# mmurooka/SMPLpp

Measured on AMD Instinct MI355X. Metric: SMPL FK evals/s + IK iters/s, batch 1024 frames, 1/2/4/8 MI355X, higher is better.
Workload: dtype f32 (exact operands: every fp32 value as three bf16 pieces = fp32's 24 bits on the bf16 matrix pipe, fp32 accumulate; fp32 VALU skinning)

## Files before the change

### smplpp_amd/csrc/fk.hip

```cpp
#include "common.h"
#include "pose_math.h"
#ifdef POSE_STAMP
namespace smplpp_hip
{
__device__ unsigned long long g_pose_stamps[16];
}
#define PST(i) if(blockIdx.x == 512 && threadIdx.x == 0) smplpp_hip::g_pose_stamps[i] = __builtin_amdgcn_s_memtime()
#define PSTC(i) if(blockIdx.x == 512 && threadIdx.x == 192) smplpp_hip::g_pose_stamps[i] = __builtin_amdgcn_s_memtime()
extern "C" int smplpp_debug_pose_stamps(unsigned long long * out)
{
  return (int)hipMemcpyFromSymbol(out, HIP_SYMBOL(smplpp_hip::g_pose_stamps), sizeof(unsigned long long) * 16);
}
#endif
#include "pose_body.h"
#include "staging.h"
#include "trace.h"

namespace smplpp_hip
{
typedef float f32x16 __attribute__((ext_vector_type(16)));
typedef _Float16 f16x8 __attribute__((ext_vector_type(8)));

__global__ __launch_bounds__(256) void pose_kernel(PoseArgs a)
{
// ... 172 lines not shown
static hipError_t launch_skin_w(const smplpp_model * m, int64_t n, const float * theta, float * verts, float * rest,
                                hipStream_t st)
{
  switch(m->maxw)
  {
    case 4:
      return launch_skin<FT, 4>(m, n, theta, verts, rest, st);
    case 8:
      return launch_skin<FT, 8>(m, n, theta, verts, rest, st);
    default:
      return launch_skin<FT, NJ>(m, n, theta, verts, rest, st);
  }
}

hipError_t launch_skin_bf16x3(const smplpp_model * m, int64_t n, const float * theta, float * verts, float * rest, hipStream_t st);
hipError_t launch_skin_f16x2(const smplpp_model * m, int64_t n, const float * theta, float * verts, float * rest, hipStream_t st);
hipError_t launch_skin_exact(const smplpp_model * m, int64_t n, const float * theta, float * verts, float * rest, hipStream_t st);

PoseArgs fk_pose_args(smplpp_model * m, int64_t n, const float * beta, const float * theta, float * joints, float * poserot, float * xforms44,
                      bool with_ops)
{
  Workspace & ws = m->ws;
  PoseArgs pa;
  pa.beta = beta;
  pa.theta = theta;
  pa.J0 = m->J0.get();
  pa.JS = m->JS.get();
  pa.JSp = m->JSp.get();
  pa.parent = m->parent.get();
  pa.lvl_off = m->lvl.get();
  pa.lvl_joint = m->lvl.get() + NJ + 1;
  pa.nlev = m->nlev;
// ... 51 lines not shown
    {
      int64_t cnt = (int64_t)KP * (ldA - n);
      zero_pad_kernel<<<dim3((unsigned)((cnt + 255) / 256)), dim3(256), 0, st>>>(ws.AT.as<float>(), ldA, n);
    }
    PoseArgs pa = fk_pose_args(m, n, beta, theta, joints, poserot, xforms44, false);
    pa.AT = ws.AT.as<float>();
    pa.ldA = ldA;
    pa.gscale = 1.0f;
    pa.range_flag = nullptr;
    pose_kernel<<<dim3((unsigned)n), dim3(256), 0, st>>>(pa);
  }
  HIP_TRY(hipGetLastError());
  return SMPLPP_OK;
}

static int fk_skin_device(smplpp_model * m, char form, int64_t n, const float * theta, float * verts, float * rest, hipStream_t st)
{
  if(verts || rest)
  {
    hipEvent_t e0 = nullptr, e1 = nullptr;
    if(m->profiling)
    {
      HIP_TRY(hipEventCreate(&e0));
      if(hipError_t ee = hipEventCreate(&e1); ee != hipSuccess)
      {
        (void)hipEventDestroy(e0);
        return hip_fail(ee, "hipEventCreate", __FILE__, __LINE__);
      }
      m->prof_events.push_back(e0);
      m->prof_events.push_back(e1);
      HIP_TRY(hipEventRecord(e0, st));
    }
    if(form == 'e')
      HIP_TRY(launch_skin_exact(m, n, theta, verts, rest, st));
    else if(form == 'h')
      HIP_TRY(launch_skin_f16x2(m, n, theta, verts, rest, st));
    else if(form == 'b')
      HIP_TRY(launch_skin_bf16x3(m, n, theta, verts, rest, st));
    else if(n <= 32)
      HIP_TRY(launch_skin_w<1>(m, n, theta, verts, rest, st));
    else
      HIP_TRY(launch_skin_w<2>(m, n, theta, verts, rest, st));
    if(m->profiling) HIP_TRY(hipEventRecord(e1, st));
  }
  return SMPLPP_OK;
}

int fk_device(smplpp_model * m, int64_t n, const float * beta, const float * theta, float * verts, float * joints,
              float * xforms44, float * rest, float * poserot, hipStream_t st, int range_slot, int * range_word, char form_override = 0)
{
  const char form = launch_form(m, range_slot, form_override);
  int rc = fk_pose_device(m, form, n, beta, theta, joints, xforms44, poserot, st, range_word ? range_word : m->range_flag.get() + range_slot,
                          verts || rest);
  if(rc) return rc;
  return fk_skin_device(m, form, n, theta, verts, rest, st);
}
}

using namespace smplpp_hip;

extern "C" int smplpp_profile_enable(smplpp_model * m, int enable)
{
  if(!m) return fail(SMPLPP_ERR_INVALID, "smplpp_profile_enable: null model");
  m->profiling = enable != 0;
  return SMPLPP_OK;
}

extern "C" int smplpp_profile_read(smplpp_model * m, int64_t * launches, double * mean_ms)
{
  if(!m || !launches || !mean_ms) return fail(SMPLPP_ERR_INVALID, "smplpp_profile_read: null argument");
// ... 77 lines not shown
```

### smplpp_amd/csrc/ik.hip

```cpp
#include "ik_types.h"
#include "ik_eval.h"
#include "ik_solve.h"
#include "ik_proj.h"
#include "vposer_state.h"

#include <algorithm>
#include <chrono>
#include <cstdlib>

using namespace smplpp_hip;

struct smplpp_ik
{
  smplpp_model * m = nullptr;
  smplpp_vposer * vp = nullptr;
  int64_t n = 0, K = 0;
  int64_t frame_base = 0;
  int theta_dim = TD75;
  TaskArrays ta{};
  float *theta = nullptr, *beta = nullptr, *theta25 = nullptr, *vjac = nullptr;
  float *verts = nullptr, *rest = nullptr, *joints = nullptr, *poserot = nullptr, *pts = nullptr;
  double *e = nullptr, *J = nullptr, *Jl = nullptr, *e2 = nullptr, *xout = nullptr;
  int *skip = nullptr, *status = nullptr, *sticky = nullptr, *list_cnt = nullptr, *list_f = nullptr;
  int * range_word = nullptr;
  int32_t * roles = nullptr;
  float * list_d = nullptr;
  std::vector<DevPtr<void>> owned;
  bool have_eval = false;
  int64_t last_D = 0;
  hipStream_t side = nullptr;
  hipEvent_t ev_fork = nullptr, ev_join = nullptr;
  bool phi_locked = false;
  bool side_pending = false;
  int * dbg_buf = nullptr;
  unsigned * sig = nullptr;
  unsigned tick_fork = 0, tick_join = 0, tick_done = 0;
  bool use_flags = false;
  double last_enqueue_us = 0.0;
  bool latent_split = false;
  bool latent_split_default = false;
  bool exact = false;
  StatePtr<VPoserJxWork> jxw;
  bool jac_ahead = false;
  bool dbg_sync = false, overlap_ok = true;
  int dbg_stop = 0;
  int64_t scan_blocks = 1536;
  int scan_form = -1;
  float * vbuf[2] = {nullptr, nullptr};
  int vcur = 0;
  ~smplpp_ik()
  {
    (void)hipSetDevice(m->device);
// ... 97 lines not shown
  if(K > PROJ_MAXK) return fail(SMPLPP_ERR_INVALID, "smplpp_ik_create: at most 48 tasks per frame are supported");
  if(TD75 + 2 * K + NB > MAXD)
    return fail(SMPLPP_ERR_INVALID, "smplpp_ik_create: too many tasks for the in-LDS solver (75 + 2K + 10 must be <= 181)");
  HIP_TRY(hipSetDevice(m->device));
  std::unique_ptr<smplpp_ik> s(new smplpp_ik());
  s->m = m;
  s->vp = vposer;
  s->n = n;
  s->K = K;
  s->theta_dim = vposer ? TD44 : TD75;
  {
    const char * e;
    s->dbg_sync = getenv("SMPLPP_DEBUG_SYNC") != nullptr;
    if((e = getenv("SMPLPP_IK_DBG_STOP"))) s->dbg_stop = atoi(e);
    if((e = getenv("SMPLPP_IK_OVERLAP"))) s->overlap_ok = e[0] != '0';
    if(s->dbg_sync) s->overlap_ok = false;
    s->scan_blocks = (n >= 256 && n < 512) ? 2 * n : 1536;
    if(n >= 512 && K <= 8 && (m->F + 767) / 768 <= 32) s->scan_blocks = n * ((m->F + 767) / 768);
    if((e = getenv("SMPLPP_SCAN_BLOCKS"))) s->scan_blocks = atoll(e);
    if((e = getenv("SMPLPP_SCAN_FORM"))) s->scan_form = atoi(e);
    s->latent_split = vposer != nullptr && n <= 128 && s->dbg_stop == 0;
    if((e = getenv("SMPLPP_IK_LATENT_SPLIT"))) s->latent_split = vposer != nullptr && e[0] != '0' && s->dbg_stop == 0;
  }
  const size_t nk = (size_t)n * K;
  const size_t Dmax = TD75 + 2 * K + NB;
  HIP_TRY(dalloc(s.get(), &s->ta.face, nk));
  HIP_TRY(dalloc(s.get(), &s->ta.vw, nk * 3));
  HIP_TRY(dalloc(s.get(), &s->ta.tang, nk * 6));
  HIP_TRY(dalloc(s.get(), &s->ta.tpos, nk * 3));
  HIP_TRY(dalloc(s.get(), &s->ta.tnrm, nk * 3));
// ... 13 lines not shown
  HIP_TRY(dalloc(s.get(), &s->rest, (size_t)n * m->V * 3));
  HIP_TRY(dalloc(s.get(), &s->joints, (size_t)n * NJ * 3));
  HIP_TRY(dalloc(s.get(), &s->poserot, (size_t)n * NJ * 9));
  HIP_TRY(dalloc(s.get(), &s->pts, nk * 3));
  HIP_TRY(dalloc(s.get(), &s->e, nk * 4));
  HIP_TRY(dalloc(s.get(), &s->J, nk * 4 * Dmax));
  HIP_TRY(dalloc(s.get(), &s->e2, (size_t)n));
  HIP_TRY(dalloc(s.get(), &s->xout, (size_t)n * Dmax));
  HIP_TRY(dalloc(s.get(), &s->roles, roles.size()));
  HIP_TRY(dalloc(s.get(), &s->list_cnt, nk));
  HIP_TRY(dalloc(s.get(), &s->list_d, nk * PROJ_LIST));
  HIP_TRY(dalloc(s.get(), &s->list_f, nk * PROJ_LIST));
  HIP_TRY(dalloc(s.get(), &s->skip, (size_t)n));
  HIP_TRY(dalloc(s.get(), &s->status, (size_t)n));
  HIP_TRY(dalloc(s.get(), &s->sticky, (size_t)n));
  HIP_TRY(dalloc(s.get(), &s->range_word, 1));
  s->ta.flags = s->sticky;
  if(vposer)
  {
    HIP_TRY(dalloc(s.get(), &s->Jl, nk * 4 * Dmax));
    HIP_TRY(dalloc(s.get(), &s->vjac, (size_t)n * 63 * 32));
  }
  auto grid = [](size_t c) { return dim3((unsigned)((c + 255) / 256)); };
  HIP_TRY(hipMemset(s->ta.face, 0, sizeof(int32_t) * nk));
  fill_f32_kernel<<<grid(nk * 3), 256>>>(s->ta.vw, 1.0f / 3.0f, nk * 3);
  fill_f32_kernel<<<grid(nk * 6), 256>>>(s->ta.tang, 0.0f, nk * 6);
  fill_f32_kernel<<<grid(nk * 3), 256>>>(s->ta.tpos, 0.0f, nk * 3);
  fill_nrm_kernel<<<grid(nk * 3), 256>>>(s->ta.tnrm, nk * 3);
  fill_f32_kernel<<<grid(nk), 256>>>(s->ta.posw, 1.0f, nk);
  fill_f32_kernel<<<grid(nk), 256>>>(s->ta.nrmw, 1.0f, nk);
  fill_f32_kernel<<<grid(nk), 256>>>(s->ta.philim, 0.04f, nk);
  fill_f32_kernel<<<grid(nk), 256>>>(s->ta.noff, 0.0f, nk);
  HIP_TRY(hipMemset(s->theta, 0, sizeof(float) * n * s->theta_dim));
  HIP_TRY(hipMemset(s->theta25, 0, sizeof(float) * n * 75));
  HIP_TRY(hipMemset(s->beta, 0, sizeof(float) * n * NB));
  HIP_TRY(hipMemset(s->skip, 0, sizeof(int) * n));
  HIP_TRY(hipMemcpy(s->roles, roles.data(), sizeof(int32_t) * roles.size(), hipMemcpyHostToDevice));
  HIP_TRY(hipMemset(s->list_cnt, 0, sizeof(int) * nk));
  HIP_TRY(hipMemset(s->status, 0, sizeof(int) * n));
  HIP_TRY(hipMemset(s->sticky, 0, sizeof(int) * n));
  HIP_TRY(hipMemset(s->range_word, 0, sizeof(int)));
  s->verts = s->vbuf[0];
  HIP_TRY(hipStreamCreateWithFlags(&s->side, hipStreamNonBlocking));
  HIP_TRY(hipEventCreateWithFlags(&s->ev_fork, hipEventDisableTiming));
  HIP_TRY(hipEventCreateWithFlags(&s->ev_join, hipEventDisableTiming));
  {
    HIP_TRY(dalloc(s.get(), &s->sig, 128));
    HIP_TRY(hipMemset(s->sig, 0, sizeof(unsigned) * 128));
    const char * e = getenv("SMPLPP_IK_EVENTS");
    if(!(e && e[0] != '0'))
    {
      s->use_flags = hipStreamWaitValue32(s->side, s->sig, 0u, hipStreamWaitValueGte, 0xffffffffu) == hipSuccess;
      (void)hipGetLastError();
    }
    if(!s->use_flags) s->latent_split = false;
    s->latent_split_default = s->latent_split;
// ... 55 lines not shown
  return SMPLPP_OK;
}

extern "C" int smplpp_ik_set_config(smplpp_ik * s, const float * beta, const float * theta, int space)
{
  if(!s) return fail(SMPLPP_ERR_INVALID, "smplpp_ik_set_config: null solver");
  int rc = check_space(space, "smplpp_ik_set_config");
  if(rc) return rc;
  HIP_TRY(hipSetDevice(s->m->device));
  hipMemcpyKind kind = space == SMPLPP_HOST ? hipMemcpyHostToDevice : hipMemcpyDeviceToDevice;
  if(beta) HIP_TRY(hipMemcpy(s->beta, beta, sizeof(float) * s->n * NB, kind));
  if(theta) HIP_TRY(hipMemcpy(s->theta, theta, sizeof(float) * s->n * s->theta_dim, kind));
  s->jac_ahead = false;
  HIP_TRY(hipMemset(s->status, 0, sizeof(int) * s->n));
  HIP_TRY(hipMemset(s->sticky, 0, sizeof(int) * s->n));
  if(s->range_word) HIP_TRY(hipMemset(s->range_word, 0, sizeof(int)));
  if(theta && s->vp)
  {
    ik_splice_kernel<<<dim3((unsigned)((s->n * 75 + 255) / 256)), 256>>>(s->theta, nullptr, s->theta25, s->n);
    HIP_TRY(hipGetLastError());
    HIP_TRY(hipStreamSynchronize(nullptr));
  }
  return SMPLPP_OK;
}

extern "C" int smplpp_ik_get_config(smplpp_ik * s, float * beta, float * theta, int space)
{
  if(!s) return fail(SMPLPP_ERR_INVALID, "smplpp_ik_get_config: null solver");
  int rc = check_space(space, "smplpp_ik_get_config");
  if(rc) return rc;
  HIP_TRY(hipSetDevice(s->m->device));
// ... 48 lines not shown
    if(s->vp && s->exact)
    {
      int rc = vposer_jacobian_device(s->vp, s->jxw, n, s->theta + 6, TD44, s->theta25 + 6, 75, s->vjac, st);
      if(rc) return rc;
      th25 = s->theta25;
    }
    else if(s->vp)
    {
      int rc = jac_elsewhere ? vposer_forward_device(s->vp, n, s->theta + 6, TD44, s->theta25 + 6, 75, nullptr, st, s->frame_base, true)
                             : vposer_forward_device(s->vp, n, s->theta + 6, TD44, s->theta25 + 6, 75, s->vjac, st, s->frame_base);
      if(rc) return rc;
      th25 = s->theta25;
    }
    s->vcur ^= 1;
    s->verts = s->vbuf[s->vcur];
    int rc = fk_device(m, n, s->beta, th25, s->verts, s->joints, nullptr, s->rest, s->poserot, st, RANGE_INTERNAL, s->range_word,
                       s->exact ? m->form : 0);
    if(rc) return rc;
  }
  TraceRange tr_eval("calculate IK matrices");
  if(s->side_pending)
  {
    if(s->use_flags)
      HIP_TRY(hipStreamWaitValue32(st, s->sig + 32, s->tick_join, hipStreamWaitValueGte, 0xffffffffu));
    else
      HIP_TRY(hipStreamWaitEvent(st, s->ev_join, 0));
    s->side_pending = false;
  }
  s->jac_ahead = false;
  const bool deep = m->nlev > 9;
  const bool wide = m->madj > MAXADJ;
  const size_t shmem = sizeof(float) * (deep ? (wide ? EvalPlan<DMAX, 64, 3>::L_END : EvalPlan<DMAX, 64, 3>::L_END)
                                             : (wide ? EvalPlan<9, 76, 4>::L_END : EvalPlan<9, 76, 6>::L_END)) + L_ANC_BYTES;
  static PerDeviceOnce once_eval[4];
  const void * kfn = deep ? (wide ? reinterpret_cast<const void *>(&ik_eval_kernel<DMAX, 64, 3, MAXADJ_WIDE>) : reinterpret_cast<const void *>(&ik_eval_kernel<DMAX, 64, 3>))
                          : (wide ? reinterpret_cast<const void *>(&ik_eval_kernel<9, 76, 4, MAXADJ_WIDE>) : reinterpret_cast<const void *>(&ik_eval_kernel<9, 76, 6>));
  HIP_TRY(lds_opt_in(once_eval[(deep ? 1 : 0) + (wide ? 2 : 0)], m->device, kfn, (int)shmem));
// ... 196 lines not shown
        int h[8];
        HIP_TRY(hipMemcpy(h, dbg_buf, sizeof(h), hipMemcpyDeviceToHost));
        fprintf(stderr, "[smplpp dbg] it %d: project lists: tasks %d, empty %d, overflow %d, nan %d, max cnt %d\n", it, h[0], h[1], h[2], h[3], h[4]);
      }
    }
    DBG_SYNC("project");
  }
#undef DBG_SYNC
  return SMPLPP_OK;
}

static int ik_join(smplpp_ik * s, hipStream_t st)
{
  if(s->side_pending)
  {
    if(s->use_flags)
      HIP_TRY(hipStreamWaitValue32(st, s->sig + 32, s->tick_join, hipStreamWaitValueGte, 0xffffffffu));
    else
      HIP_TRY(hipStreamWaitEvent(st, s->ev_join, 0));
    s->side_pending = false;
  }
  return SMPLPP_OK;
}

static int ik_check_status(smplpp_ik * s, const int * flags)
{
  std::vector<int> h((size_t)s->n);
  HIP_TRY(hipMemcpy(h.data(), flags, sizeof(int) * s->n, hipMemcpyDeviceToHost));
  for(int64_t f = 0; f < s->n; f++)
    if(h[f] & 1) return fail(SMPLPP_ERR_NUMERIC, "LLT has numerical issue!");
  return SMPLPP_OK;
}

static int ik_check_valence(smplpp_ik * s)
{
  std::vector<int> h((size_t)s->n);
  HIP_TRY(hipMemcpy(h.data(), s->sticky, sizeof(int) * s->n, hipMemcpyDeviceToHost));
  for(int64_t f = 0; f < s->n; f++)
    if(h[f] & 4)
      return fail(SMPLPP_ERR_INVALID, "a task with a normal term (normal weight or normal offset) touches a vertex with more than 12 adjacent "
                                      "faces: the Jacobian of such a term is not supported");
  return SMPLPP_OK;
}

extern "C" int smplpp_ik_iterate(smplpp_ik * s, int iters, int enable_qp, int optimize_beta_from, int64_t min_valid,
// ... 28 lines not shown
}

__global__ void ik_seq_frame_kernel(const float * __restrict__ tpos_t, const uint8_t * __restrict__ valid_t, float * __restrict__ tpos,
                                    float * __restrict__ posw, int64_t nk, const float * __restrict__ theta, float * __restrict__ theta_prev_out,
                                    int64_t ntheta, int64_t shared_K)
{
  const int64_t i = (int64_t)blockIdx.x * blockDim.x + threadIdx.x;
  if(tpos_t && i < nk)
  {
    const int64_t j = shared_K > 0 ? i % shared_K : i;
    const bool v = valid_t[j] != 0;
    posw[i] = v ? 1.0f : 0.0f;
    for(int x = 0; x < 3; x++) tpos[i * 3 + x] = v ? tpos_t[j * 3 + x] : 0.0f;
  }
  if(theta_prev_out && i < ntheta) theta_prev_out[i] = theta[i];
}

extern "C" int smplpp_debug_ik_enqueue_us(smplpp_ik * s, double * out)
{
  if(!s || !out) return fail(SMPLPP_ERR_INVALID, "smplpp_debug_ik_enqueue_us: bad argument");
  *out = s->last_enqueue_us;
  return SMPLPP_OK;
}

static int ik_solve_sequence_impl(smplpp_ik * s, int64_t T, const float * target_pos, const uint8_t * valid, bool shared, int warmup_iters,
                                  int iters_per_frame, int enable_qp, int64_t min_valid, float * theta_out, int space, void * stream)
{
  if(!s || T <= 0 || !target_pos || !valid || !theta_out || warmup_iters < 0 || iters_per_frame < 0)
    return fail(SMPLPP_ERR_INVALID, "smplpp_ik_solve_sequence: bad argument");
  int rc = check_space(space, "smplpp_ik_solve_sequence");
  if(rc) return rc;
  HIP_TRY(hipSetDevice(s->m->device));
  hipStream_t st = static_cast<hipStream_t>(stream);
  const int64_t nk = s->n * s->K, ntheta = s->n * s->theta_dim;
  const int64_t tk = shared ? s->K : nk;
  In<float> tp;
  In<uint8_t> vl;
  Out<float> th;
  HIP_TRY(tp.init(target_pos, (size_t)(T * tk * 3), space, st));
  HIP_TRY(vl.init(valid, (size_t)(T * tk), space, st));
  HIP_TRY(th.init(theta_out, (size_t)(T * ntheta), space));
  HIP_TRY(hipMemsetAsync(s->sticky, 0, sizeof(int) * s->n, st));
  const int64_t cnt = nk > ntheta ? nk : ntheta;
  const dim3 grid((unsigned)((cnt + 255) / 256));
  ik_seq_frame_kernel<<<grid, 256, 0, st>>>(tp.d, vl.d, s->ta.tpos, s->ta.posw, nk, nullptr, nullptr, 0, shared ? s->K : 0);
  HIP_TRY(hipGetLastError());
  const auto enq_t0 = std::chrono::steady_clock::now();
  for(int64_t t = 0; t < T; t++)
  {
    const int iters = t == 0 ? warmup_iters : iters_per_frame;
    SeqHook hook;
    hook.theta_record = th.d + t * ntheta;
    if(t + 1 < T)
    {
      hook.next_tpos = tp.d + (t + 1) * tk * 3;
      hook.next_valid = vl.d + (t + 1) * tk;
      hook.shared = shared ? 1 : 0;
// ... 34 lines not shown
{
  return ik_solve_sequence_impl(s, T, target_pos, valid, true, warmup_iters, iters_per_frame, enable_qp, min_valid, theta_out, space, stream);
}

extern "C" int smplpp_ik_get_status(smplpp_ik * s, int32_t * flags, int space, void * stream)
{
  if(!s || !flags) return fail(SMPLPP_ERR_INVALID, "smplpp_ik_get_status: bad argument");
  int rc = check_space(space, "smplpp_ik_get_status");
  if(rc) return rc;
  HIP_TRY(hipSetDevice(s->m->device));
  hipStream_t st = static_cast<hipStream_t>(stream);
  std::vector<int> a((size_t)s->n), b((size_t)s->n);
  HIP_TRY(hipStreamSynchronize(st));
  HIP_TRY(hipMemcpy(a.data(), s->status, sizeof(int) * s->n, hipMemcpyDeviceToHost));
  HIP_TRY(hipMemcpy(b.data(), s->sticky, sizeof(int) * s->n, hipMemcpyDeviceToHost));
  int internal = 0;
  if(s->range_word && s->m->form_ik == 'h') HIP_TRY(hipMemcpy(&internal, s->range_word, sizeof(int), hipMemcpyDeviceToHost));
  std::vector<int32_t> h((size_t)s->n);
  for(int64_t f = 0; f < s->n; f++)
    h[(size_t)f] = (a[(size_t)f] == 1 ? 1 : 0) | ((b[(size_t)f] & 1) ? 2 : 0) | (b[(size_t)f] & 4) | ((internal & 1) ? 8 : 0) |
                   (a[(size_t)f] == 2 ? 16 : 0);
  if(space == SMPLPP_HOST)
    memcpy(flags, h.data(), sizeof(int32_t) * (size_t)s->n);
  else
    HIP_TRY(hipMemcpy(flags, h.data(), sizeof(int32_t) * (size_t)s->n, hipMemcpyHostToDevice));
  return SMPLPP_OK;
}

extern "C" int smplpp_ik_get_step(smplpp_ik * s, double * x, int64_t * D, int space, void * stream)
{
  if(!s || !D) return fail(SMPLPP_ERR_INVALID, "smplpp_ik_get_step: bad argument");
  int rc = check_space(space, "smplpp_ik_get_step");
  if(rc) return rc;
  *D = s->last_D;
  if(!x || s->last_D == 0) return SMPLPP_OK;
  HIP_TRY(hipSetDevice(s->m->device));
// ... 21 lines not shown
```

### smplpp_amd/csrc/ik_types.h

```cpp
#pragma once
#include "mesh_device.h"
#include "staging.h"
#include "trace.h"
#include "signal.h"

#include <hip/hip_ext.h>

struct smplpp_vposer;

namespace smplpp_hip
{
int fk_device(smplpp_model * m, int64_t n, const float * beta, const float * theta, float * verts, float * joints,
              float * xforms44, float * rest, float * poserot, hipStream_t st, int range_slot, int * range_word = nullptr,
              char form_override = 0);
int vposer_forward_device(smplpp_vposer * v, int64_t n, const float * z, int64_t z_stride, float * out, int64_t out_stride,
                          float * jac, hipStream_t st, int64_t frame_base, bool value_like_jac = false, unsigned * sig_flag = nullptr,
                          unsigned * sig_counter = nullptr, unsigned sig_tick = 0u);

constexpr int TD75 = SMPLPP_THETA_DIM;
constexpr int TD44 = SMPLPP_LATENT_POSE_DIM;
constexpr int NQ = TD75 + NB;
constexpr int IK_MAXK = 48;
constexpr size_t SOLVE_LDS_MAX = 160 * 1024 - 1536;
constexpr int MAXD = TD75 + 2 * IK_MAXK + NB;

struct TaskArrays
{
  int32_t * face;
  float * vw;
// ... 57 lines not shown
```

### smplpp_amd/csrc/signal.h

```cpp
#pragma once
#include <hip/hip_runtime.h>

namespace smplpp_hip
{
template<class T>
__device__ inline void st_agent(T * p, T v)
{
  __hip_atomic_store(p, v, __ATOMIC_RELAXED, __HIP_MEMORY_SCOPE_AGENT);
}
__device__ inline void wg_signal(unsigned * __restrict__ flag, unsigned * __restrict__ counter, unsigned tick)
{
  if(!flag) return;
  asm volatile("s_waitcnt vmcnt(0)" ::: "memory");
  __syncthreads();
  if(threadIdx.x == 0)
  {
    if(__hip_atomic_fetch_add(counter, 1u, __ATOMIC_RELAXED, __HIP_MEMORY_SCOPE_AGENT) == gridDim.x - 1)
    {
      __hip_atomic_store(counter, 0u, __ATOMIC_RELAXED, __HIP_MEMORY_SCOPE_AGENT);
      __hip_atomic_store(flag, tick, __ATOMIC_RELAXED, __HIP_MEMORY_SCOPE_SYSTEM);
    }
  }
}

}
```

### smplpp_amd/csrc/skin_e.hip

```cpp
#include "common.h"
#include "slot_pipe.h"

namespace smplpp_hip
{
typedef float f32x16 __attribute__((ext_vector_type(16)));
typedef float v3f __attribute__((ext_vector_type(3), aligned(4)));
typedef float v4f __attribute__((ext_vector_type(4)));
typedef int v4i __attribute__((ext_vector_type(4)));
typedef unsigned v3u __attribute__((ext_vector_type(3)));
typedef __bf16 bf16x8 __attribute__((ext_vector_type(8)));

constexpr int E_R = 4;
constexpr int E_G_BYTES = 64 * NJ * 48;
constexpr int E_LDS_RING = E_G_BYTES;
constexpr int E_LDS_ROOT = E_LDS_RING + E_R * EB_IMG;
constexpr int E_LDS_TOTAL = E_LDS_ROOT + 64 * 16;
constexpr int E_SLOTS = 18;
constexpr int E_NSLOT = EB_KS * E_SLOTS;
constexpr int E_BAR = 6;
constexpr int E_NDMA = 5;
constexpr int E_PITCH = 13;
constexpr int E_ROW0 = 12;
constexpr int E_ROW_END = E_ROW0 + 15 * E_PITCH + 13;
#ifndef SKINE_RD_AHEAD
// ... 84 lines not shown
static_assert(E_LDS_TOTAL <= 160 * 1024, "LDS plan");
static_assert(E_ROW_END < 12 * E_SLOTS + E_BAR, "the rows end before the slots a run's first item uses for its G' DMAs");
static_assert(E_ROW0 + 1 - E_RD_AHEAD > E_BAR, "the first G' read of an item follows the barrier that publishes the tile");
static_assert(E_GDMA0 + E_GCHUNKS <= E_NSLOT, "the G' DMAs fit the item");
static_assert(e_barrier_vmcnt(0, true, false) == 5 && (E_A_PRE != 4 || (e_barrier_vmcnt(1, false, false) == 10 + 3 && e_barrier_vmcnt(3, false, false) == 10 + 9 && e_barrier_vmcnt(5, false, false) == 10 + 9 && e_barrier_vmcnt(13, false, false) == 10 + 17)) &&
                  e_barrier_vmcnt(3, true, false) == 10 + 3 && e_barrier_vmcnt(5, true, false) == 10 + 4,
              "window bookkeeping");

#if SKINE_ABL & 512
__device__ unsigned long long g_ewg_times[256 * 8];
#endif
#if SKINE_ABL & 256
__device__ unsigned long long g_eslot_times[8 * 256];
#endif

template<int MAXW, bool WANT_REST>
__global__ __launch_bounds__(256, 1) void skin_kernel_e(const uint8_t * __restrict__ A3, const uint8_t * __restrict__ B3e,
                                                        const float * __restrict__ Gp, const float * __restrict__ theta,
                                                        float * __restrict__ verts, float * __restrict__ rest, int64_t n, int64_t V,
                                                        int nvg, int nft)
{
  extern __shared__ __attribute__((aligned(16))) unsigned char lds[];
  typedef __attribute__((address_space(3))) void * lds_ptr_t;
  const int tid = threadIdx.x, lane = tid & 63, half = lane >> 5, l31 = lane & 31;
  const int wave = __builtin_amdgcn_readfirstlane(tid >> 6), wf = wave & 1, wv = wave >> 1;
  const int nbx = (int)(gridDim.x >> 3), xcd = (int)(blockIdx.x & 7), jb = (int)(blockIdx.x >> 3);
  const int vg0 = (xcd * nvg) >> 3, vg1 = ((xcd + 1) * nvg) >> 3, nvx = vg1 - vg0;
  const int cnt = nvx * nft;
  const int i0 = (int)(((unsigned)jb * (unsigned)cnt) / (unsigned)nbx), i1 = (int)(((unsigned)(jb + 1) * (unsigned)cnt) / (unsigned)nbx);
  if(i0 >= i1) return;
#if SKINE_ABL & 512
  const unsigned long long t_start = __builtin_amdgcn_s_memtime(), r_start = __builtin_amdgcn_s_memrealtime();
  unsigned long long t_first = 0, t_last = 0, t_drain0 = 0, t_run2 = 0;
#endif

  const int frameB = (int)(V * 12);
  const __amdgpu_buffer_rsrc_t rsB = __builtin_amdgcn_make_buffer_rsrc(const_cast<uint8_t *>(B3e), 0, (int)(nvg * EB_KS * EB_IMG), 0x00020000);
  const __amdgpu_buffer_rsrc_t rsG = __builtin_amdgcn_make_buffer_rsrc(const_cast<float *>(Gp), 0, (int)(nft * E_G_BYTES), 0x00020000);
  const __amdgpu_buffer_rsrc_t rsV = __builtin_amdgcn_make_buffer_rsrc(verts, 0, (int)(verts ? n * V * 12 : 0), 0x00020000);
  const __amdgpu_buffer_rsrc_t rsR = __builtin_amdgcn_make_buffer_rsrc(rest, 0, (int)(rest ? n * V * 12 : 0), 0x00020000);
  const int voffDma = wave * (E_NDMA * 1024) + lane * 16;
  const int voffG = tid * 16;

  const unsigned char * imgV[E_R];
  int imgS[E_R];
// ... 367 lines not shown
  drain();
#if SKINE_ABL & 512
  if(tid == 0 && blockIdx.x < 256)
  {
    g_ewg_times[blockIdx.x * 8 + 0] = r_start;
    g_ewg_times[blockIdx.x * 8 + 1] = __builtin_amdgcn_s_memrealtime();
    g_ewg_times[blockIdx.x * 8 + 2] = __builtin_amdgcn_s_memtime() - t_start;
    g_ewg_times[blockIdx.x * 8 + 3] = (unsigned long long)(i1 - i0);
    g_ewg_times[blockIdx.x * 8 + 4] = t_first - t_start;
    g_ewg_times[blockIdx.x * 8 + 5] = __builtin_amdgcn_s_memtime() - t_last;
    g_ewg_times[blockIdx.x * 8 + 6] = t_run2 ? t_run2 - t_drain0 : 0;
    g_ewg_times[blockIdx.x * 8 + 7] = t_last - t_first;
  }
#endif
  asm volatile("s_waitcnt vmcnt(0)" ::: "memory");
}

template<int MAXW, bool WANT_REST>
static hipError_t launch_e(const smplpp_model * m, int64_t n, const float * theta, float * verts, float * rest, hipStream_t st, int64_t f_off)
{
  const int nft = (int)((n + 63) / 64);
  const int nvg = (int)m->VGPn;
  const int per_xcd_items = ((nvg + 7) / 8) * nft;
  int nbx = device_cus(m->device) / 8;
  if(nbx > per_xcd_items) nbx = per_xcd_items;
  if(nbx < 1) nbx = 1;
  {
    const int rounds = (per_xcd_items + nbx - 1) / nbx;
    nbx = (per_xcd_items + rounds - 1) / rounds;
  }
  static PerDeviceOnce once;
  {
    hipError_t e = lds_opt_in(once, m->device, reinterpret_cast<const void *>(&skin_kernel_e<MAXW, WANT_REST>), E_LDS_TOTAL);
    if(e != hipSuccess) return e;
  }
  skin_kernel_e<MAXW, WANT_REST><<<dim3(nbx * 8), dim3(256), E_LDS_TOTAL, st>>>(
      m->ws.A3.as<uint8_t>() + (f_off / 64) * (int64_t)(BB_KS * BB_A_BYTES), m->B3e.get(), m->ws.Gp.as<float>() + f_off * (NJ * 12),
      theta + f_off * ((NJ + 1) * 3), verts ? verts + f_off * m->V * 3 : nullptr, rest ? rest + f_off * m->V * 3 : nullptr, n, m->V, nvg, nft);
  return hipGetLastError();
}

#if SKINE_ABL & 256
extern "C" int smplpp_debug_eslot_times(unsigned long long * out)
{
  return (int)hipMemcpyFromSymbol(out, HIP_SYMBOL(smplpp_hip::g_eslot_times), sizeof(unsigned long long) * 8 * 256);
}
#endif
#if SKINE_ABL & 512
extern "C" int smplpp_debug_ewg_times(unsigned long long * out)
{
  return (int)hipMemcpyFromSymbol(out, HIP_SYMBOL(smplpp_hip::g_ewg_times), sizeof(unsigned long long) * 256 * 8);
}
#endif
hipError_t launch_skin_exact(const smplpp_model * m, int64_t n, const float * theta, float * verts, float * rest, hipStream_t st)
{
  int64_t per = (0x7fffff00LL / (m->V * 12)) & ~63LL;
  const int64_t per_g = (0x7fffff00LL / E_G_BYTES) * 64;
  if(per > per_g) per = per_g;
  if(per < 64) return hipErrorInvalidValue;
  for(int64_t off = 0; off < n; off += per)
  {
    const int64_t nn = (n - off < per) ? n - off : per;
    hipError_t e = rest ? launch_e<4, true>(m, nn, theta, verts, rest, st, off) : launch_e<4, false>(m, nn, theta, verts, rest, st, off);
    if(e != hipSuccess) return e;
  }
  return hipSuccess;
}
}
```

### smplpp_amd/csrc/skin_h.hip

```cpp
#include "common.h"
#include "slot_pipe.h"

namespace smplpp_hip
{
typedef float f32x16 __attribute__((ext_vector_type(16)));
typedef float v3f __attribute__((ext_vector_type(3), aligned(4)));
typedef float v4f __attribute__((ext_vector_type(4)));
typedef unsigned v3u __attribute__((ext_vector_type(3)));
typedef _Float16 f16x8 __attribute__((ext_vector_type(8)));

constexpr int H_R = 7;
constexpr int H_LDS_RING = HB_G_BYTES;
constexpr int H_LDS_TR = H_LDS_RING + H_R * HB_IMG;
constexpr int H_LDS_TOTAL = H_LDS_TR + 64 * 16;

constexpr int wrap15(int u)
{
  return u < 0 ? u + HB_SLOTS : u;
}
constexpr int h_tail_slot(int k)
{
  return k <= 4 ? k : (k == 5 ? 4 : (k <= 10 ? k - 1 : (k == 11 ? 9 : k - 2)));
}
constexpr int h_tail_m(int k)
// ... 28 lines not shown

#ifndef SKINH_STORE_AUX
#define SKINH_STORE_AUX 0
#endif
#ifndef SKINH_DMA_IMM
#define SKINH_DMA_IMM 1
#endif
#ifndef SKINH_ABL
#define SKINH_ABL 0
#endif
#if SKINH_ABL & (256 | 512)
__device__ unsigned long long g_hslot_times[8 * 256];
__device__ unsigned long long g_hwg_times[256 * 4];
#endif

template<bool WANT_REST>
__global__ __launch_bounds__(256, 1) void skin_kernel_h(const uint8_t * __restrict__ A2h, const uint8_t * __restrict__ B2h,
                                                        const uint8_t * __restrict__ G2h, const float * __restrict__ theta,
                                                        float * __restrict__ verts, float * __restrict__ rest, int64_t n,
                                                        int64_t V, int nvg, int nft, float cAB)
{
  extern __shared__ __attribute__((aligned(16))) unsigned char lds[];
  typedef __attribute__((address_space(3))) void * lds_ptr_t;
  const int tid = threadIdx.x, lane = tid & 63, half = lane >> 5, l31 = lane & 31;
  const int wave = __builtin_amdgcn_readfirstlane(tid >> 6), wf = wave & 1, wv = wave >> 1;
  const int nbx = (int)(gridDim.x >> 3), xcd = (int)(blockIdx.x & 7), jb = (int)(blockIdx.x >> 3);
  const int vg0 = (xcd * nvg) >> 3, vg1 = ((xcd + 1) * nvg) >> 3, nvx = vg1 - vg0;
  const int cnt = nvx * nft;
  const int i0 = (int)(((unsigned)jb * (unsigned)cnt) / (unsigned)nbx), i1 = (int)(((unsigned)(jb + 1) * (unsigned)cnt) / (unsigned)nbx);
  if(i0 >= i1) return;

#if SKINH_ABL & 512
  const unsigned long long t_start = __builtin_amdgcn_s_memtime(), r_start = __builtin_amdgcn_s_memrealtime();
#endif
  const int frameB = (int)(V * 12);
  const __amdgpu_buffer_rsrc_t rsB =
      __builtin_amdgcn_make_buffer_rsrc(const_cast<uint8_t *>(B2h), 0, (int)(nvg * HB_SLOTS * HB_IMG), 0x00020000);
  const __amdgpu_buffer_rsrc_t rsG =
      __builtin_amdgcn_make_buffer_rsrc(const_cast<uint8_t *>(G2h), 0, (int)(nft * HB_G_BYTES), 0x00020000);
  const __amdgpu_buffer_rsrc_t rsV = __builtin_amdgcn_make_buffer_rsrc(verts, 0, (int)(verts ? n * V * 12 : 0), 0x00020000);
  const __amdgpu_buffer_rsrc_t rsR = __builtin_amdgcn_make_buffer_rsrc(rest, 0, (int)(rest ? n * V * 12 : 0), 0x00020000);
  const int voffDma = wave * 3072 + lane * 16;

  const unsigned char * imgV[H_R];
  int imgS[H_R];
// ... 332 lines not shown
    g_hslot_times[64] = __builtin_amdgcn_s_memtime();
    g_hslot_times[65] = __builtin_amdgcn_s_memrealtime();
    g_hslot_times[66] = t_start;
    g_hslot_times[67] = r_start;
    g_hslot_times[68] = i1 - i0;
  }
  if(tid == 0 && blockIdx.x < 256)
  {
    g_hwg_times[blockIdx.x * 4 + 0] = r_start;
    g_hwg_times[blockIdx.x * 4 + 1] = __builtin_amdgcn_s_memrealtime();
    g_hwg_times[blockIdx.x * 4 + 2] = __builtin_amdgcn_s_memtime() - t_start;
    g_hwg_times[blockIdx.x * 4 + 3] = (unsigned long long)(i1 - i0) | ((unsigned long long)__builtin_amdgcn_s_getreg((6 << 11) | 20) << 32);
  }
#endif
  asm volatile("s_waitcnt vmcnt(0)" ::: "memory");
}

static hipError_t launch_h(const smplpp_model * m, int64_t n, const float * theta, float * verts, float * rest, hipStream_t st,
                           int64_t f_off)
{
  const int nft = (int)((n + 63) / 64);
  const int nvg = (int)m->VGPn;
  const int per_xcd_items = ((nvg + 7) / 8) * nft;
  int nbx = device_cus(m->device) / 8;
  if(nbx > per_xcd_items) nbx = per_xcd_items;
  if(nbx < 1) nbx = 1;
  {
    const int rounds = (per_xcd_items + nbx - 1) / nbx;
    nbx = (per_xcd_items + rounds - 1) / rounds;
  }
  const bool wr = rest != nullptr;
  static PerDeviceOnce once[2];
  {
    hipError_t e = lds_opt_in(once[wr], m->device, wr ? reinterpret_cast<const void *>(&skin_kernel_h<true>) : reinterpret_cast<const void *>(&skin_kernel_h<false>), H_LDS_TOTAL);
    if(e != hipSuccess) return e;
  }
  const float cAB = 1.0f / (HB_SA * m->sB);
  const uint8_t * A2 = m->ws.A2h.as<uint8_t>() + (f_off / 64) * (int64_t)(HB_KS * HB_A_BYTES);
  const uint8_t * G2 = m->ws.G2h.as<uint8_t>() + (f_off / 64) * (int64_t)HB_G_BYTES;
  const float * th = theta + f_off * ((NJ + 1) * 3);
  float * vo = verts ? verts + f_off * m->V * 3 : nullptr;
  float * ro = rest ? rest + f_off * m->V * 3 : nullptr;
  if(wr)
    skin_kernel_h<true><<<dim3(nbx * 8), dim3(256), H_LDS_TOTAL, st>>>(A2, m->B2h.get(), G2, th, vo, ro, n, m->V, nvg, nft, cAB);
  else
    skin_kernel_h<false><<<dim3(nbx * 8), dim3(256), H_LDS_TOTAL, st>>>(A2, m->B2h.get(), G2, th, vo, ro, n, m->V, nvg, nft, cAB);
  return hipGetLastError();
}

#if SKINH_ABL & (256 | 512)
extern "C" int smplpp_debug_hwg_times(unsigned long long * out)
{
  return (int)hipMemcpyFromSymbol(out, HIP_SYMBOL(smplpp_hip::g_hwg_times), sizeof(unsigned long long) * 256 * 4);
}
extern "C" int smplpp_debug_hslot_times(unsigned long long * out)
{
  return (int)hipMemcpyFromSymbol(out, HIP_SYMBOL(smplpp_hip::g_hslot_times), sizeof(unsigned long long) * 8 * 256);
}
#endif
hipError_t launch_skin_f16x2(const smplpp_model * m, int64_t n, const float * theta, float * verts, float * rest, hipStream_t st)
{
  int64_t per = (0x7fffff00LL / (m->V * 12)) & ~63LL;
  const int64_t per_g = (0x7fffff00LL / HB_G_BYTES) * 64;
  if(per > per_g) per = per_g;
  if(per < 64) return hipErrorInvalidValue;
  for(int64_t off = 0; off < n; off += per)
  {
    const int64_t nn = (n - off < per) ? n - off : per;
    hipError_t e = launch_h(m, nn, theta, verts, rest, st, off);
    if(e != hipSuccess) return e;
  }
  return hipSuccess;
}
}
```

Measured before the change: 15.11 million.

## Fold side-stream join wait into the skinning kernel tail instead of a stream wait packet

Within an IK iteration, the wait on the side re-projection stream used to be a hipStreamWaitValue32 packet on the main stream. It now runs inside the last skinning kernel launch: after that block finishes its work, thread 0 of block 0 spin-waits on the signal flag. This is meant to remove the separate wait packet and its queue-processing gap between kernels. The spin wait has a time budget, and an expired wait sets a status bit that is checked later. If the wait runs out, the join is not actually enforced, and the spinning block holds a CU slot.

```diff
diff --git a/smplpp_amd/csrc/fk.hip b/smplpp_amd/csrc/fk.hip
--- a/smplpp_amd/csrc/fk.hip
+++ b/smplpp_amd/csrc/fk.hip
@@ -1,4 +1,5 @@
 #include "common.h"
+#include "signal.h"
 #include "pose_math.h"
 #ifdef POSE_STAMP
 namespace smplpp_hip
@@ -210,8 +211,10 @@
 }
 
 hipError_t launch_skin_bf16x3(const smplpp_model * m, int64_t n, const float * theta, float * verts, float * rest, hipStream_t st);
-hipError_t launch_skin_f16x2(const smplpp_model * m, int64_t n, const float * theta, float * verts, float * rest, hipStream_t st);
-hipError_t launch_skin_exact(const smplpp_model * m, int64_t n, const float * theta, float * verts, float * rest, hipStream_t st);
+hipError_t launch_skin_f16x2(const smplpp_model * m, int64_t n, const float * theta, float * verts, float * rest, hipStream_t st,
+                             JoinWait * join = nullptr);
+hipError_t launch_skin_exact(const smplpp_model * m, int64_t n, const float * theta, float * verts, float * rest, hipStream_t st,
+                             JoinWait * join = nullptr);
 
 PoseArgs fk_pose_args(smplpp_model * m, int64_t n, const float * beta, const float * theta, float * joints, float * poserot, float * xforms44,
                       bool with_ops)
@@ -293,7 +296,8 @@
   return SMPLPP_OK;
 }
 
-static int fk_skin_device(smplpp_model * m, char form, int64_t n, const float * theta, float * verts, float * rest, hipStream_t st)
+static int fk_skin_device(smplpp_model * m, char form, int64_t n, const float * theta, float * verts, float * rest, hipStream_t st,
+                          JoinWait * join)
 {
   if(verts || rest)
   {
@@ -311,9 +315,9 @@
       HIP_TRY(hipEventRecord(e0, st));
     }
     if(form == 'e')
-      HIP_TRY(launch_skin_exact(m, n, theta, verts, rest, st));
+      HIP_TRY(launch_skin_exact(m, n, theta, verts, rest, st, join));
     else if(form == 'h')
-      HIP_TRY(launch_skin_f16x2(m, n, theta, verts, rest, st));
+      HIP_TRY(launch_skin_f16x2(m, n, theta, verts, rest, st, join));
     else if(form == 'b')
       HIP_TRY(launch_skin_bf16x3(m, n, theta, verts, rest, st));
     else if(n <= 32)
@@ -326,13 +330,19 @@
 }
 
 int fk_device(smplpp_model * m, int64_t n, const float * beta, const float * theta, float * verts, float * joints,
-              float * xforms44, float * rest, float * poserot, hipStream_t st, int range_slot, int * range_word, char form_override = 0)
+              float * xforms44, float * rest, float * poserot, hipStream_t st, int range_slot, int * range_word, char form_override,
+              JoinWait * join)
 {
   const char form = launch_form(m, range_slot, form_override);
   int rc = fk_pose_device(m, form, n, beta, theta, joints, xforms44, poserot, st, range_word ? range_word : m->range_flag.get() + range_slot,
                           verts || rest);
   if(rc) return rc;
-  return fk_skin_device(m, form, n, theta, verts, rest, st);
+  return fk_skin_device(m, form, n, theta, verts, rest, st, join);
+}
+int fk_device(smplpp_model * m, int64_t n, const float * beta, const float * theta, float * verts, float * joints,
+              float * xforms44, float * rest, float * poserot, hipStream_t st, int range_slot, int * range_word, char form_override = 0)
+{
+  return fk_device(m, n, beta, theta, verts, joints, xforms44, rest, poserot, st, range_slot, range_word, form_override, nullptr);
 }
 }
 
diff --git a/smplpp_amd/csrc/ik.hip b/smplpp_amd/csrc/ik.hip
--- a/smplpp_amd/csrc/ik.hip
+++ b/smplpp_amd/csrc/ik.hip
@@ -7,6 +7,7 @@
 #include <algorithm>
 #include <chrono>
 #include <cstdlib>
+#include <cstring>
 
 using namespace smplpp_hip;
 
@@ -23,6 +24,7 @@
   double *e = nullptr, *J = nullptr, *Jl = nullptr, *e2 = nullptr, *xout = nullptr;
   int *skip = nullptr, *status = nullptr, *sticky = nullptr, *list_cnt = nullptr, *list_f = nullptr;
   int * range_word = nullptr;
+  int * join_word = nullptr;
   int32_t * roles = nullptr;
   float * list_d = nullptr;
   std::vector<DevPtr<void>> owned;
@@ -36,6 +38,8 @@
   unsigned * sig = nullptr;
   unsigned tick_fork = 0, tick_join = 0, tick_done = 0;
   bool use_flags = false;
+  bool join_in_kernel = true;
+  int64_t join_counts[3] = {0, 0, 0};
   double last_enqueue_us = 0.0;
   bool latent_split = false;
   bool latent_split_default = false;
@@ -163,6 +167,11 @@
     s->dbg_sync = getenv("SMPLPP_DEBUG_SYNC") != nullptr;
     if((e = getenv("SMPLPP_IK_DBG_STOP"))) s->dbg_stop = atoi(e);
     if((e = getenv("SMPLPP_IK_OVERLAP"))) s->overlap_ok = e[0] != '0';
+    if((e = getenv("SMPLPP_IK_JOIN")))
+    {
+      if(strcmp(e, "kernel") != 0 && strcmp(e, "packet") != 0) return fail(SMPLPP_ERR_INVALID, "smplpp_ik_create: SMPLPP_IK_JOIN is kernel or packet");
+      s->join_in_kernel = strcmp(e, "kernel") == 0;
+    }
     if(s->dbg_sync) s->overlap_ok = false;
     s->scan_blocks = (n >= 256 && n < 512) ? 2 * n : 1536;
     if(n >= 512 && K <= 8 && (m->F + 767) / 768 <= 32) s->scan_blocks = n * ((m->F + 767) / 768);
@@ -206,7 +215,8 @@
   HIP_TRY(dalloc(s.get(), &s->skip, (size_t)n));
   HIP_TRY(dalloc(s.get(), &s->status, (size_t)n));
   HIP_TRY(dalloc(s.get(), &s->sticky, (size_t)n));
-  HIP_TRY(dalloc(s.get(), &s->range_word, 1));
+  HIP_TRY(dalloc(s.get(), &s->range_word, 2));
+  s->join_word = s->range_word + 1;
   s->ta.flags = s->sticky;
   if(vposer)
   {
@@ -231,7 +241,7 @@
   HIP_TRY(hipMemset(s->list_cnt, 0, sizeof(int) * nk));
   HIP_TRY(hipMemset(s->status, 0, sizeof(int) * n));
   HIP_TRY(hipMemset(s->sticky, 0, sizeof(int) * n));
-  HIP_TRY(hipMemset(s->range_word, 0, sizeof(int)));
+  HIP_TRY(hipMemset(s->range_word, 0, sizeof(int) * 2));
   s->verts = s->vbuf[0];
   HIP_TRY(hipStreamCreateWithFlags(&s->side, hipStreamNonBlocking));
   HIP_TRY(hipEventCreateWithFlags(&s->ev_fork, hipEventDisableTiming));
@@ -317,7 +327,7 @@
   s->jac_ahead = false;
   HIP_TRY(hipMemset(s->status, 0, sizeof(int) * s->n));
   HIP_TRY(hipMemset(s->sticky, 0, sizeof(int) * s->n));
-  if(s->range_word) HIP_TRY(hipMemset(s->range_word, 0, sizeof(int)));
+  if(s->range_word) HIP_TRY(hipMemset(s->range_word, 0, sizeof(int) * 2));
   if(theta && s->vp)
   {
     ik_splice_kernel<<<dim3((unsigned)((s->n * 75 + 255) / 256)), 256>>>(s->theta, nullptr, s->theta25, s->n);
@@ -396,13 +406,27 @@
     }
     s->vcur ^= 1;
     s->verts = s->vbuf[s->vcur];
+    JoinWait jw;
+    const bool kjoin = s->side_pending && s->use_flags && s->join_in_kernel && !s->latent_split && !s->jac_ahead && s->dbg_stop == 0 && !s->dbg_sync;
+    if(kjoin)
+    {
+      jw.flag = s->sig + 32;
+      jw.tick = s->tick_join;
+      jw.status = s->join_word;
+    }
     int rc = fk_device(m, n, s->beta, th25, s->verts, s->joints, nullptr, s->rest, s->poserot, st, RANGE_INTERNAL, s->range_word,
-                       s->exact ? m->form : 0);
+                       s->exact ? m->form : 0, kjoin ? &jw : nullptr);
     if(rc) return rc;
+    if(jw.carried)
+    {
+      s->side_pending = false;
+      s->join_counts[0]++;
+    }
   }
   TraceRange tr_eval("calculate IK matrices");
   if(s->side_pending)
   {
+    s->join_counts[1]++;
     if(s->use_flags)
       HIP_TRY(hipStreamWaitValue32(st, s->sig + 32, s->tick_join, hipStreamWaitValueGte, 0xffffffffu));
     else
@@ -629,6 +653,7 @@
 {
   if(s->side_pending)
   {
+    s->join_counts[2]++;
     if(s->use_flags)
       HIP_TRY(hipStreamWaitValue32(st, s->sig + 32, s->tick_join, hipStreamWaitValueGte, 0xffffffffu));
     else
@@ -644,6 +669,9 @@
   HIP_TRY(hipMemcpy(h.data(), flags, sizeof(int) * s->n, hipMemcpyDeviceToHost));
   for(int64_t f = 0; f < s->n; f++)
     if(h[f] & 1) return fail(SMPLPP_ERR_NUMERIC, "LLT has numerical issue!");
+  int joined = 0;
+  HIP_TRY(hipMemcpy(&joined, s->join_word, sizeof(int), hipMemcpyDeviceToHost));
+  if(joined & JOIN_EXPIRED) return fail(SMPLPP_ERR_NUMERIC, "an IK iteration's wait for its re-projection stream ran out of its time budget");
   return SMPLPP_OK;
 }
 
@@ -702,6 +730,13 @@
     for(int x = 0; x < 3; x++) tpos[i * 3 + x] = v ? tpos_t[j * 3 + x] : 0.0f;
   }
   if(theta_prev_out && i < ntheta) theta_prev_out[i] = theta[i];
+}
+
+extern "C" int smplpp_debug_ik_join_counts(smplpp_ik * s, int64_t * out)
+{
+  if(!s || !out) return fail(SMPLPP_ERR_INVALID, "smplpp_debug_ik_join_counts: bad argument");
+  for(int i = 0; i < 3; i++) out[i] = s->join_counts[i];
+  return SMPLPP_OK;
 }
 
 extern "C" int smplpp_debug_ik_enqueue_us(smplpp_ik * s, double * out)
@@ -729,6 +764,7 @@
   HIP_TRY(vl.init(valid, (size_t)(T * tk), space, st));
   HIP_TRY(th.init(theta_out, (size_t)(T * ntheta), space));
   HIP_TRY(hipMemsetAsync(s->sticky, 0, sizeof(int) * s->n, st));
+  HIP_TRY(hipMemsetAsync(s->join_word, 0, sizeof(int), st));
   const int64_t cnt = nk > ntheta ? nk : ntheta;
   const dim3 grid((unsigned)((cnt + 255) / 256));
   ik_seq_frame_kernel<<<grid, 256, 0, st>>>(tp.d, vl.d, s->ta.tpos, s->ta.posw, nk, nullptr, nullptr, 0, shared ? s->K : 0);
@@ -793,12 +829,13 @@
   HIP_TRY(hipStreamSynchronize(st));
   HIP_TRY(hipMemcpy(a.data(), s->status, sizeof(int) * s->n, hipMemcpyDeviceToHost));
   HIP_TRY(hipMemcpy(b.data(), s->sticky, sizeof(int) * s->n, hipMemcpyDeviceToHost));
-  int internal = 0;
+  int internal = 0, joined = 0;
   if(s->range_word && s->m->form_ik == 'h') HIP_TRY(hipMemcpy(&internal, s->range_word, sizeof(int), hipMemcpyDeviceToHost));
+  HIP_TRY(hipMemcpy(&joined, s->join_word, sizeof(int), hipMemcpyDeviceToHost));
   std::vector<int32_t> h((size_t)s->n);
   for(int64_t f = 0; f < s->n; f++)
     h[(size_t)f] = (a[(size_t)f] == 1 ? 1 : 0) | ((b[(size_t)f] & 1) ? 2 : 0) | (b[(size_t)f] & 4) | ((internal & 1) ? 8 : 0) |
-                   (a[(size_t)f] == 2 ? 16 : 0);
+                   ((joined & JOIN_EXPIRED) ? 32 : 0) | (a[(size_t)f] == 2 ? 16 : 0);
   if(space == SMPLPP_HOST)
     memcpy(flags, h.data(), sizeof(int32_t) * (size_t)s->n);
   else
diff --git a/smplpp_amd/csrc/ik_types.h b/smplpp_amd/csrc/ik_types.h
--- a/smplpp_amd/csrc/ik_types.h
+++ b/smplpp_amd/csrc/ik_types.h
@@ -13,6 +13,9 @@
 int fk_device(smplpp_model * m, int64_t n, const float * beta, const float * theta, float * verts, float * joints,
               float * xforms44, float * rest, float * poserot, hipStream_t st, int range_slot, int * range_word = nullptr,
               char form_override = 0);
+int fk_device(smplpp_model * m, int64_t n, const float * beta, const float * theta, float * verts, float * joints,
+              float * xforms44, float * rest, float * poserot, hipStream_t st, int range_slot, int * range_word, char form_override,
+              JoinWait * join);
 int vposer_forward_device(smplpp_vposer * v, int64_t n, const float * z, int64_t z_stride, float * out, int64_t out_stride,
                           float * jac, hipStream_t st, int64_t frame_base, bool value_like_jac = false, unsigned * sig_flag = nullptr,
                           unsigned * sig_counter = nullptr, unsigned sig_tick = 0u);
diff --git a/smplpp_amd/csrc/signal.h b/smplpp_amd/csrc/signal.h
--- a/smplpp_amd/csrc/signal.h
+++ b/smplpp_amd/csrc/signal.h
@@ -23,4 +23,27 @@
   }
 }
 
+struct JoinWait
+{
+  const unsigned * flag = nullptr;
+  unsigned tick = 0;
+  int * status = nullptr;
+  bool carried = false;
+};
+constexpr unsigned long long JOIN_WAIT_BUDGET_TICKS = 400000ull;
+constexpr int JOIN_EXPIRED = 1;
+__device__ inline void join_wait(const unsigned * __restrict__ flag, unsigned tick, int * __restrict__ status)
+{
+  const unsigned long long t0 = __builtin_amdgcn_s_memrealtime();
+  while(__hip_atomic_load(flag, __ATOMIC_ACQUIRE, __HIP_MEMORY_SCOPE_AGENT) < tick)
+  {
+    if(__builtin_amdgcn_s_memrealtime() - t0 > JOIN_WAIT_BUDGET_TICKS)
+    {
+      __hip_atomic_fetch_or(status, JOIN_EXPIRED, __ATOMIC_RELAXED, __HIP_MEMORY_SCOPE_AGENT);
+      return;
+    }
+    __builtin_amdgcn_s_sleep(2);
+  }
 }
+
+}
diff --git a/smplpp_amd/csrc/skin_e.hip b/smplpp_amd/csrc/skin_e.hip
--- a/smplpp_amd/csrc/skin_e.hip
+++ b/smplpp_amd/csrc/skin_e.hip
@@ -1,4 +1,5 @@
 #include "common.h"
+#include "signal.h"
 #include "slot_pipe.h"
 
 namespace smplpp_hip
@@ -122,11 +123,11 @@
 __device__ unsigned long long g_eslot_times[8 * 256];
 #endif
 
-template<int MAXW, bool WANT_REST>
+template<int MAXW, bool WANT_REST, class... JOIN>
 __global__ __launch_bounds__(256, 1) void skin_kernel_e(const uint8_t * __restrict__ A3, const uint8_t * __restrict__ B3e,
                                                         const float * __restrict__ Gp, const float * __restrict__ theta,
                                                         float * __restrict__ verts, float * __restrict__ rest, int64_t n, int64_t V,
-                                                        int nvg, int nft)
+                                                        int nvg, int nft, JOIN... join)
 {
   extern __shared__ __attribute__((aligned(16))) unsigned char lds[];
   typedef __attribute__((address_space(3))) void * lds_ptr_t;
@@ -136,7 +137,15 @@
   const int vg0 = (xcd * nvg) >> 3, vg1 = ((xcd + 1) * nvg) >> 3, nvx = vg1 - vg0;
   const int cnt = nvx * nft;
   const int i0 = (int)(((unsigned)jb * (unsigned)cnt) / (unsigned)nbx), i1 = (int)(((unsigned)(jb + 1) * (unsigned)cnt) / (unsigned)nbx);
-  if(i0 >= i1) return;
+  auto carry_join = [&]() {
+    if constexpr(sizeof...(JOIN) != 0)
+      if(blockIdx.x == 0 && threadIdx.x == 0) join_wait(join...);
+  };
+  if(i0 >= i1)
+  {
+    carry_join();
+    return;
+  }
 #if SKINE_ABL & 512
   const unsigned long long t_start = __builtin_amdgcn_s_memtime(), r_start = __builtin_amdgcn_s_memrealtime();
   unsigned long long t_first = 0, t_last = 0, t_drain0 = 0, t_run2 = 0;
@@ -534,10 +543,12 @@
   }
 #endif
   asm volatile("s_waitcnt vmcnt(0)" ::: "memory");
+  carry_join();
 }
 
 template<int MAXW, bool WANT_REST>
-static hipError_t launch_e(const smplpp_model * m, int64_t n, const float * theta, float * verts, float * rest, hipStream_t st, int64_t f_off)
+static hipError_t launch_e(const smplpp_model * m, int64_t n, const float * theta, float * verts, float * rest, hipStream_t st, int64_t f_off,
+                           JoinWait * join)
 {
   const int nft = (int)((n + 63) / 64);
   const int nvg = (int)m->VGPn;
@@ -554,9 +565,24 @@
     hipError_t e = lds_opt_in(once, m->device, reinterpret_cast<const void *>(&skin_kernel_e<MAXW, WANT_REST>), E_LDS_TOTAL);
     if(e != hipSuccess) return e;
   }
-  skin_kernel_e<MAXW, WANT_REST><<<dim3(nbx * 8), dim3(256), E_LDS_TOTAL, st>>>(
-      m->ws.A3.as<uint8_t>() + (f_off / 64) * (int64_t)(BB_KS * BB_A_BYTES), m->B3e.get(), m->ws.Gp.as<float>() + f_off * (NJ * 12),
-      theta + f_off * ((NJ + 1) * 3), verts ? verts + f_off * m->V * 3 : nullptr, rest ? rest + f_off * m->V * 3 : nullptr, n, m->V, nvg, nft);
+  const uint8_t * const A3 = m->ws.A3.as<uint8_t>() + (f_off / 64) * (int64_t)(BB_KS * BB_A_BYTES);
+  const float * const Gp = m->ws.Gp.as<float>() + f_off * (NJ * 12);
+  const float * const th = theta + f_off * ((NJ + 1) * 3);
+  float * const vo = verts ? verts + f_off * m->V * 3 : nullptr;
+  float * const ro = rest ? rest + f_off * m->V * 3 : nullptr;
+  if constexpr(WANT_REST)
+    if(join && join->flag)
+    {
+      static PerDeviceOnce once_join;
+      hipError_t e = lds_opt_in(once_join, m->device,
+                                reinterpret_cast<const void *>(&skin_kernel_e<MAXW, true, const unsigned *, unsigned, int *>), E_LDS_TOTAL);
+      if(e != hipSuccess) return e;
+      skin_kernel_e<MAXW, true, const unsigned *, unsigned, int *><<<dim3(nbx * 8), dim3(256), E_LDS_TOTAL, st>>>(
+          A3, m->B3e.get(), Gp, th, vo, ro, n, m->V, nvg, nft, join->flag, join->tick, join->status);
+      join->carried = true;
+      return hipGetLastError();
+    }
+  skin_kernel_e<MAXW, WANT_REST><<<dim3(nbx * 8), dim3(256), E_LDS_TOTAL, st>>>(A3, m->B3e.get(), Gp, th, vo, ro, n, m->V, nvg, nft);
   return hipGetLastError();
 }
 
@@ -572,7 +598,8 @@
   return (int)hipMemcpyFromSymbol(out, HIP_SYMBOL(smplpp_hip::g_ewg_times), sizeof(unsigned long long) * 256 * 8);
 }
 #endif
-hipError_t launch_skin_exact(const smplpp_model * m, int64_t n, const float * theta, float * verts, float * rest, hipStream_t st)
+hipError_t launch_skin_exact(const smplpp_model * m, int64_t n, const float * theta, float * verts, float * rest, hipStream_t st,
+                             JoinWait * join)
 {
   int64_t per = (0x7fffff00LL / (m->V * 12)) & ~63LL;
   const int64_t per_g = (0x7fffff00LL / E_G_BYTES) * 64;
@@ -581,7 +608,8 @@
   for(int64_t off = 0; off < n; off += per)
   {
     const int64_t nn = (n - off < per) ? n - off : per;
-    hipError_t e = rest ? launch_e<4, true>(m, nn, theta, verts, rest, st, off) : launch_e<4, false>(m, nn, theta, verts, rest, st, off);
+    JoinWait * const jw = off + nn >= n ? join : nullptr;
+    hipError_t e = rest ? launch_e<4, true>(m, nn, theta, verts, rest, st, off, jw) : launch_e<4, false>(m, nn, theta, verts, rest, st, off, jw);
     if(e != hipSuccess) return e;
   }
   return hipSuccess;
diff --git a/smplpp_amd/csrc/skin_h.hip b/smplpp_amd/csrc/skin_h.hip
--- a/smplpp_amd/csrc/skin_h.hip
+++ b/smplpp_amd/csrc/skin_h.hip
@@ -1,4 +1,5 @@
 #include "common.h"
+#include "signal.h"
 #include "slot_pipe.h"
 
 namespace smplpp_hip
@@ -66,11 +67,11 @@
 __device__ unsigned long long g_hwg_times[256 * 4];
 #endif
 
-template<bool WANT_REST>
+template<bool WANT_REST, class... JOIN>
 __global__ __launch_bounds__(256, 1) void skin_kernel_h(const uint8_t * __restrict__ A2h, const uint8_t * __restrict__ B2h,
                                                         const uint8_t * __restrict__ G2h, const float * __restrict__ theta,
                                                         float * __restrict__ verts, float * __restrict__ rest, int64_t n,
-                                                        int64_t V, int nvg, int nft, float cAB)
+                                                        int64_t V, int nvg, int nft, float cAB, JOIN... join)
 {
   extern __shared__ __attribute__((aligned(16))) unsigned char lds[];
   typedef __attribute__((address_space(3))) void * lds_ptr_t;
@@ -80,7 +81,15 @@
   const int vg0 = (xcd * nvg) >> 3, vg1 = ((xcd + 1) * nvg) >> 3, nvx = vg1 - vg0;
   const int cnt = nvx * nft;
   const int i0 = (int)(((unsigned)jb * (unsigned)cnt) / (unsigned)nbx), i1 = (int)(((unsigned)(jb + 1) * (unsigned)cnt) / (unsigned)nbx);
-  if(i0 >= i1) return;
+  auto carry_join = [&]() {
+    if constexpr(sizeof...(JOIN) != 0)
+      if(blockIdx.x == 0 && threadIdx.x == 0) join_wait(join...);
+  };
+  if(i0 >= i1)
+  {
+    carry_join();
+    return;
+  }
 
 #if SKINH_ABL & 512
   const unsigned long long t_start = __builtin_amdgcn_s_memtime(), r_start = __builtin_amdgcn_s_memrealtime();
@@ -443,10 +452,11 @@
   }
 #endif
   asm volatile("s_waitcnt vmcnt(0)" ::: "memory");
+  carry_join();
 }
 
 static hipError_t launch_h(const smplpp_model * m, int64_t n, const float * theta, float * verts, float * rest, hipStream_t st,
-                           int64_t f_off)
+                           int64_t f_off, JoinWait * join)
 {
   const int nft = (int)((n + 63) / 64);
   const int nvg = (int)m->VGPn;
@@ -459,9 +469,14 @@
     nbx = (per_xcd_items + rounds - 1) / rounds;
   }
   const bool wr = rest != nullptr;
-  static PerDeviceOnce once[2];
-  {
-    hipError_t e = lds_opt_in(once[wr], m->device, wr ? reinterpret_cast<const void *>(&skin_kernel_h<true>) : reinterpret_cast<const void *>(&skin_kernel_h<false>), H_LDS_TOTAL);
+  const bool jn = wr && join && join->flag;
+  static PerDeviceOnce once[3];
+  {
+    hipError_t e = lds_opt_in(once[jn ? 2 : wr], m->device,
+                              jn   ? reinterpret_cast<const void *>(&skin_kernel_h<true, const unsigned *, unsigned, int *>)
+                              : wr ? reinterpret_cast<const void *>(&skin_kernel_h<true>)
+                                   : reinterpret_cast<const void *>(&skin_kernel_h<false>),
+                              H_LDS_TOTAL);
     if(e != hipSuccess) return e;
   }
   const float cAB = 1.0f / (HB_SA * m->sB);
@@ -470,7 +485,13 @@
   const float * th = theta + f_off * ((NJ + 1) * 3);
   float * vo = verts ? verts + f_off * m->V * 3 : nullptr;
   float * ro = rest ? rest + f_off * m->V * 3 : nullptr;
-  if(wr)
+  if(jn)
+  {
+    skin_kernel_h<true, const unsigned *, unsigned, int *><<<dim3(nbx * 8), dim3(256), H_LDS_TOTAL, st>>>(
+        A2, m->B2h.get(), G2, th, vo, ro, n, m->V, nvg, nft, cAB, join->flag, join->tick, join->status);
+    join->carried = true;
+  }
+  else if(wr)
     skin_kernel_h<true><<<dim3(nbx * 8), dim3(256), H_LDS_TOTAL, st>>>(A2, m->B2h.get(), G2, th, vo, ro, n, m->V, nvg, nft, cAB);
   else
     skin_kernel_h<false><<<dim3(nbx * 8), dim3(256), H_LDS_TOTAL, st>>>(A2, m->B2h.get(), G2, th, vo, ro, n, m->V, nvg, nft, cAB);
@@ -487,7 +508,8 @@
   return (int)hipMemcpyFromSymbol(out, HIP_SYMBOL(smplpp_hip::g_hslot_times), sizeof(unsigned long long) * 8 * 256);
 }
 #endif
-hipError_t launch_skin_f16x2(const smplpp_model * m, int64_t n, const float * theta, float * verts, float * rest, hipStream_t st)
+hipError_t launch_skin_f16x2(const smplpp_model * m, int64_t n, const float * theta, float * verts, float * rest, hipStream_t st,
+                             JoinWait * join)
 {
   int64_t per = (0x7fffff00LL / (m->V * 12)) & ~63LL;
   const int64_t per_g = (0x7fffff00LL / HB_G_BYTES) * 64;
@@ -496,7 +518,7 @@
   for(int64_t off = 0; off < n; off += per)
   {
     const int64_t nn = (n - off < per) ? n - off : per;
-    hipError_t e = launch_h(m, nn, theta, verts, rest, st, off);
+    hipError_t e = launch_h(m, nn, theta, verts, rest, st, off, off + nn >= n ? join : nullptr);
     if(e != hipSuccess) return e;
   }
   return hipSuccess;
```

Result: no change. 14.98 million (-0.8%).
